# cv-core/MIT-Driverless-CV-TrainingInfra

Measured on AMD Instinct MI355X. Metric: images/sec training (YOLOv3 416^2 + RektNet 80^2), higher is better.
Workload: dtype bf16; 1 GPU; CVC-YOLOv3 yolo_baseline 416x416 classes=80, train step (fwd+bwd+Adam), 32 img/GPU; global_batch=32, parallelism=dp1, hipgraph=False, optimizer=FusedAdam

## Files before the change

### include/mdcv_hip.h

```cpp
#ifndef MDCV_HIP_H
#define MDCV_HIP_H
#ifdef __cplusplus
extern "C" {
#endif

#define MDCV_OK 0
#define MDCV_EARG (-1)
#define MDCV_F32 0
#define MDCV_BF16 1
#define MDCV_TUNED(dtype, code) (((dtype) & 0xff) | ((code) * 256))
#define MDCV_ACT_NONE 0
#define MDCV_ACT_LEAKY 1
#define MDCV_ACT_RELU 2

int mdcv_conv2d(int dtype, int mode, const void* in, int in_ldc, const void* w_packed, void* out, int out_ldc,
                const float* bias, const void* addsrc, int add_ldc, float* stats_partial,
                int B, int Hin, int Win, int Cin, int Hout, int Wout, int Nout,
                int KH, int KW, int stride, int pad, int dil, void* stream);
int mdcv_conv2d_affine_act(int dtype, const void* in, int in_ldc, const void* w_packed, void* out, int out_ldc, const float* scale,
                           const float* shift, const void* addsrc, int add_ldc, int act, float slope, int B, int Hin, int Win, int Cin,
                           int Hout, int Wout, int Nout, int KH, int KW, int stride, int pad, int dil, void* stream);
int mdcv_conv2d_dgrad_bnsums_rows(int dtype, int B, int Hin, int Win, int Cin, int Hout, int Wout, int Nout, int KH, int KW, int stride,
                                  int pad, int dil, int in_ldc);
int mdcv_conv2d_dgrad_bnsums(int dtype, const void* in, int in_ldc, const void* w_packed, void* out, int out_ldc, const void* addsrc,
// ... 162 lines not shown
int mdcv_event_destroy(void* ev);
int mdcv_probe_mfma(int blocks, int iters, float* sink, double* flops, void* stream);
int mdcv_stream_fork(void* from, void* to, int device_scope);
int mdcv_stream_fork_arm(void* from, int device_scope, void** ev_out);
int mdcv_stream_fork_wait(void* to, void* ev);
int mdcv_profile_begin(void);
int mdcv_profile_count(void);
int mdcv_profile_stop(void);
int mdcv_profile_read(int i, float* ms, char* name, int name_len);
int mdcv_graph_begin(void* stream);
int mdcv_graph_end(void* stream, void** graph_exec);
int mdcv_graph_launch(void* graph_exec, void* stream);
int mdcv_graph_destroy(void* graph_exec);

int mdcv_pw_rows(long long M, int K);
int mdcv_pw_conv_fwd(int dtype, const void* y, int ldy, const float* scale, const float* shift, const void* resid, int ldr, int act,
                     float slope, void* z_out, int ldz, const void* w_packed, const float* bias, void* out, int out_ldc,
                     float* stats_partial, long long M, int K, int N, void* stream);

int mdcv_pw_bwd_slabs(int dtype, long long M, int Cin, int Cout, int ldy, int ldx, int lddx, int ldadd, int ldfy);
int mdcv_pw_bwd(int dtype, const void* dy, int ldy, const void* x, int ldx, const void* wd_packed, void* dx, int lddx, const void* addsrc,
                int ldadd, float* ws, int slabs, const void* fy, int ldfy, const float* fscale, const float* fshift, const float* fmean, int fact,
                float fslope, float* fpartial, long long M, int Cin, int Cout, void* stream);
int mdcv_conv2d_wgrad_bnapply_ok(int dtype, int B, int Hin, int Win, int Cin, int Hout, int Wout, int Cout, int KH, int KW, int stride,
                                 int pad, int dil, int dz_ldc, int y_ldc, int x_ldc);
int mdcv_conv2d_wgrad_bnapply(int dtype, const void* dz, int dz_ldc, const void* y, int y_ldc, const float* scale, const float* shift,
                              const float* cA, const float* cB, const float* cC, int act, float slope, const void* x, int x_ldc, float* ws,
                              int splits, float* dw_oihw, int accumulate, int B, int Hin, int Win, int Cin, int Cin_real, int Hout, int Wout,
                              int Cout, int Cout_real, int KH, int KW, int stride, int pad, int dil, void* stream);
int mdcv_wgrad_reduce(const float* ws, int splits, float* dw_oihw, int accumulate, int Cout_pad, int Cout, int Cin_pad, int Cin, int KK,
                      void* stream);

int mdcv_comm_unique_id(void* id128);
int mdcv_comm_init(void** comm, int nranks, const void* id128, int rank);
int mdcv_comm_allreduce_sum(void* comm, float* buf, long long n, void* stream);
int mdcv_comm_destroy(void* comm);

#ifdef __cplusplus
}
#endif
#endif
```

### mit-driverless-cv-traininginfra_amd/csrc/pw_bwd.hip

```cpp
#include "common.h"
#include "bn_fuse.h"

struct PwbArgs {
  const void* dy; const void* x; const void* wd; void* dx; const void* addsrc; float* ws;
  int ldy, ldx, lddx, ldadd;
  int M, Cin, Cout;
  int slab_px, nslabs, slices;
  BnFuseArgs fuse;
};

namespace {

constexpr int NT = 512, NW = 8;
constexpr int BP = 32;
constexpr int NS = 64;
constexpr int T64 = 2 * 2048 + 128;
constexpr int SPITCH = 136;
typedef __attribute__((address_space(3))) void lds_void_t;
typedef __attribute__((ext_vector_type(4))) short s16x4_t;
typedef __attribute__((ext_vector_type(8))) short s16x8_t;


__device__ __forceinline__ int swz(int row) { return (row >> 1) & 2; }
__device__ __forceinline__ unsigned lds_u32(const unsigned char* p) {
  return (unsigned)(size_t)(const __attribute__((address_space(3))) unsigned char*)p;
}
__device__ __forceinline__ uint2 lds_rd64(unsigned addr) {
  uint2 v;
  asm volatile("ds_read_b64 %0, %1" : "=v"(v) : "v"(addr) : "memory");
  return v;
}
template <int OFF> __device__ __forceinline__ s16x4_t lds_tr16(unsigned addr) {
  s16x4_t v;
  asm volatile("ds_read_b64_tr_b16 %0, %1 offset:%2" : "=v"(v) : "v"(addr), "n"(OFF) : "memory");
  return v;
}

template <int CO4, int S, bool ADD, bool FUSE>
__global__ __launch_bounds__(NT) void pw_bwd_kernel(PwbArgs a) {
  constexpr int KB = 2 * CO4;
  constexpr int NX = 1 + (ADD ? 1 : 0) + (FUSE ? 1 : 0);
  constexpr int WD_BYTES = KB * 4096;
  constexpr int STG = KB * 2048 + NX * T64;
  constexpr int STAGING = WD_BYTES + S * STG;
  constexpr int DUMP = STAGING + BP * SPITCH;
  constexpr int NCHUNK = 2 * KB + 4 * NX;
  constexpr int NPW = (NCHUNK + NW - 1) / NW;
  extern __shared__ __attribute__((aligned(1024))) unsigned char smem[];

  const int xcd = (int)(blockIdx.x & 7), seq = (int)(blockIdx.x >> 3);
  const int slab = xcd + 8 * (seq / a.slices), slice = seq % a.slices;
  if (slab >= a.nslabs) return;
  const int tid = threadIdx.x, lane = tid & 63;
  const int wave = __builtin_amdgcn_readfirstlane(tid >> 6);
  const int px0 = slab * a.slab_px;
  const int px_end = min(a.M, px0 + a.slab_px);
  const int ntiles = (px_end - px0 + BP - 1) / BP;
  const int ci0 = slice * NS;

  const __amdgpu_buffer_rsrc_t rwd = __builtin_amdgcn_make_buffer_rsrc(const_cast<void*>(a.wd), 0, (unsigned)a.Cin * (unsigned)a.Cout * 2u, 0x00020000);

  const int lrow = lane >> 2, lslot = (lane & 3) ^ swz(lrow);
#define PWB_SETUP(I)                                                                                                               \
  const int c##I = wave + NW * I;                                                                                 \
  const int cc##I = c##I - 2 * KB, t##I = cc##I >> 2, b##I = (cc##I >> 1) & 1, g##I = c##I & 1;                                      \
  const bool isdy##I = c##I < 2 * KB, live##I = c##I < NCHUNK;                                                                       \
  const int k##I = isdy##I ? 0 : (t##I == 0 ? 1 : ((ADD && t##I == 1) ? 2 : 3));                      \
  const void* bp##I = k##I == 0 ? a.dy : (k##I == 1 ? a.x : (k##I == 2 ? a.addsrc : a.fuse.y));                                     \
  const unsigned ld##I = (unsigned)(k##I == 0 ? a.ldy : (k##I == 1 ? a.ldx : (k##I == 2 ? a.ldadd : a.fuse.ldy)));                  \
  const unsigned pitch##I = live##I ? ld##I * 2u : 0u;                                                                              \
  const __amdgpu_buffer_rsrc_t rs##I = __builtin_amdgcn_make_buffer_rsrc(const_cast<void*>(live##I ? bp##I : a.dy), 0,              \
                                                                         live##I ? (unsigned)px_end * ld##I * 2u : 0u, 0x00020000); \
  const int ch##I = isdy##I ? (c##I >> 1) * 32 : ci0 + b##I * 32;                                                                   \
  const unsigned voff##I = live##I ? (unsigned)(g##I * 16 + lrow) * pitch##I + (unsigned)(ch##I + lslot * 8) * 2u : 0u;             \
  const unsigned ldso##I = !live##I ? (unsigned)(DUMP - WD_BYTES)                                                                   \
                                    : (isdy##I ? (unsigned)((c##I >> 1) * 2048 + g##I * 1024)                                       \
                                               : (unsigned)(KB * 2048 + t##I * T64 + b##I * (2048 + 128) + g##I * 1024));           \
  const unsigned smul##I = live##I ? (unsigned)STG : 0u;
  PWB_SETUP(0) PWB_SETUP(1) PWB_SETUP(2) PWB_SETUP(3) PWB_SETUP(4) PWB_SETUP(5)
#undef PWB_SETUP
  static_assert(NPW <= 6, "six DMA roles per wave");
#define PWB_ISSUE_ONE(I, PROW_, SLOT_)                                                                                             \
  if constexpr (I < NPW)                                                                                                          \
    __builtin_amdgcn_raw_ptr_buffer_load_lds(rs##I, (lds_void_t*)(smem + WD_BYTES + (unsigned)(SLOT_) * smul##I + ldso##I), 16,      \
                                             (int)voff##I, (int)((PROW_) * pitch##I), 0, 0)
#define PWB_ISSUE_TILE(T_, SLOT_)                                                                                                  \
  do {                                                                                                                           \
    const unsigned prow__ = (unsigned)(px0 + (T_) * BP);                                                                         \
    PWB_ISSUE_ONE(0, prow__, SLOT_); PWB_ISSUE_ONE(1, prow__, SLOT_); PWB_ISSUE_ONE(2, prow__, SLOT_);                           \
    PWB_ISSUE_ONE(3, prow__, SLOT_); PWB_ISSUE_ONE(4, prow__, SLOT_); PWB_ISSUE_ONE(5, prow__, SLOT_);                           \
  } while (0)

#pragma unroll
  for (int i = 0; i < (4 * KB) / NW; ++i) {
    const int c = wave + NW * i, kb = c >> 2, g = c & 3;
    const unsigned vo = (unsigned)(ci0 + g * 16 + lrow) * (unsigned)a.Cout * 2u + (unsigned)(kb * 32 + lslot * 8) * 2u;
    __builtin_amdgcn_raw_ptr_buffer_load_lds(rwd, (lds_void_t*)(smem + kb * 4096 + g * 1024), 16, (int)vo, 0, 0, 0);
  }
  int issued = 0;
  for (; issued < S - 1 && issued < ntiles; ++issued) PWB_ISSUE_TILE(issued, issued);

  const int r16 = lane & 15, q4 = lane >> 4;
  const int offF = r16 * 64 + ((q4 ^ swz(r16)) << 4);
  const int cb = wave & 3, pb = wave >> 2;
  const unsigned char* const pWd = smem + (cb * 16) * 64 + offF;
  const int trow = q4 * 4 + (r16 >> 2);
  const int tsub = (r16 & 1) * 8, tq = (r16 & 3) >> 1;
  const int wc = wave >> 1, wn = wave & 1;
  const int erow = tid >> 4, ecg = tid & 15;
  const int eblk = ecg >> 3, eslot = (ecg & 7) >> 1, esub = (ecg & 1) * 8;
  const int eoff64 = eblk * (2048 + 128) + erow * 64 + ((eslot ^ swz(erow & 15)) << 4) + esub;
  bf16_t* __restrict__ dxp = reinterpret_cast<bf16_t*>(a.dx);
  const unsigned stg_wr = lds_u32(smem) + (unsigned)(STAGING + (pb * 16 + r16) * SPITCH + cb * 32 + q4 * 8);

  float fs[4], fb[4], fm[4], sg[4], sx[4];
  if constexpr (FUSE) {
#pragma unroll
    for (int e = 0; e < 4; ++e) {
      const int n = ci0 + ecg * 4 + e;
      fs[e] = a.fuse.scale[n]; fb[e] = a.fuse.shift[n]; fm[e] = a.fuse.mean[n]; sg[e] = 0.f; sx[e] = 0.f;
    }
  }

  f32x4_t accw[CO4][2];
#pragma unroll
  for (int i = 0; i < CO4; ++i)
#pragma unroll
    for (int j = 0; j < 2; ++j) accw[i][j] = f32x4_t{0.f, 0.f, 0.f, 0.f};

  int slot = 0, islot = issued % S;
  for (int t = 0; t < ntiles; ++t) {
    const int newer = issued - 1 - t;
    if (S > 2 && newer >= S - 2) asm volatile("s_waitcnt vmcnt(%0)" ::"n"((S > 2 ? S - 2 : 0) * NPW) : "memory");
    else asm volatile("s_waitcnt vmcnt(0)" ::: "memory");
    asm volatile("s_waitcnt lgkmcnt(0)" ::: "memory");
    __builtin_amdgcn_s_barrier();
    if (issued < ntiles) {
      PWB_ISSUE_TILE(issued, islot);
      ++issued;
      islot = islot + 1 == S ? 0 : islot + 1;
    }
    const unsigned char* stg = smem + WD_BYTES + slot * STG;

    {
      f32x4_t acc = f32x4_t{0.f, 0.f, 0.f, 0.f};
      const unsigned char* pB = stg + (pb * 16) * 64 + offF;
#pragma unroll
      for (int kb = 0; kb < KB; ++kb) {
        const bf16x8_t fa = *reinterpret_cast<const bf16x8_t*>(pWd + kb * 4096);
        const bf16x8_t fbv = *reinterpret_cast<const bf16x8_t*>(pB + kb * 2048);
        acc = __builtin_amdgcn_mfma_f32_16x16x32_bf16(fa, fbv, acc, 0, 0, 0);
      }
      uint2 pk;
      pk.x = pack_bf16x2(acc[0], acc[1]); pk.y = pack_bf16x2(acc[2], acc[3]);
      asm volatile("ds_write_b64 %0, %1" ::"v"(stg_wr), "v"(pk) : "memory");
    }

    {
      bf16x8_t fx[2], fd[CO4];
      const unsigned xb = lds_u32(stg) + (unsigned)(KB * 2048 + wn * (2048 + 128) + trow * 64 + tsub);
#pragma unroll
      for (int j = 0; j < 2; ++j) {
        const unsigned ad = xb + (unsigned)((((2 * j + tq) ^ swz(trow)) << 4));
        const s16x4_t lo = lds_tr16<0>(ad), hi = lds_tr16<1024>(ad);
        const s16x8_t v = {lo[0], lo[1], lo[2], lo[3], hi[0], hi[1], hi[2], hi[3]};
        fx[j] = __builtin_bit_cast(bf16x8_t, v);
      }
      const unsigned db = lds_u32(stg) + (unsigned)(trow * 64 + tsub);
#pragma unroll
      for (int i = 0; i < CO4; ++i) {
        const int gblk = wc * CO4 + i;
        const unsigned ad = db + (unsigned)((gblk >> 1) * 2048) + (unsigned)((((2 * (gblk & 1) + tq) ^ swz(trow)) << 4));
        const s16x4_t lo = lds_tr16<0>(ad), hi = lds_tr16<1024>(ad);
        const s16x8_t v = {lo[0], lo[1], lo[2], lo[3], hi[0], hi[1], hi[2], hi[3]};
        fd[i] = __builtin_bit_cast(bf16x8_t, v);
      }
      asm volatile("s_waitcnt lgkmcnt(0)" ::: "memory");
#pragma unroll
      for (int j = 0; j < 2; ++j) asm volatile("" : "+v"(fx[j]));
#pragma unroll
      for (int i = 0; i < CO4; ++i) asm volatile("" : "+v"(fd[i]));
#pragma unroll
      for (int i = 0; i < CO4; ++i)
#pragma unroll
        for (int j = 0; j < 2; ++j) accw[i][j] = __builtin_amdgcn_mfma_f32_16x16x32_bf16(fd[i], fx[j], accw[i][j], 0, 0, 0);
    }

    asm volatile("s_waitcnt lgkmcnt(0)" ::: "memory");
    __builtin_amdgcn_s_barrier();
    {
      const int p = px0 + t * BP + erow;
      const unsigned sbase = lds_u32(stg) + (unsigned)(KB * 2048 + eoff64);
      uint2 d = lds_rd64(lds_u32(smem) + (unsigned)(STAGING + erow * SPITCH + ecg * 8)), q = d, yq = d;
      if constexpr (ADD) q = lds_rd64(sbase + T64);
      if constexpr (FUSE) yq = lds_rd64(sbase + (NX - 1) * T64);
      asm volatile("s_waitcnt lgkmcnt(0)" : "+v"(d), "+v"(q), "+v"(yq)::"memory");
      float v[4];
      v[0] = __uint_as_float(d.x << 16); v[1] = __uint_as_float(d.x & 0xffff0000u);
      v[2] = __uint_as_float(d.y << 16); v[3] = __uint_as_float(d.y & 0xffff0000u);
      if constexpr (ADD) {
        v[0] += __uint_as_float(q.x << 16); v[1] += __uint_as_float(q.x & 0xffff0000u);
        v[2] += __uint_as_float(q.y << 16); v[3] += __uint_as_float(q.y & 0xffff0000u);
        d.x = pack_bf16x2(v[0], v[1]); d.y = pack_bf16x2(v[2], v[3]);
      }
      if (p < px_end) *reinterpret_cast<uint2*>(dxp + (size_t)p * a.lddx + ci0 + ecg * 4) = d;
      if constexpr (FUSE) {
        if (p < px_end) {
          float yv[4];
          yv[0] = __uint_as_float(yq.x << 16); yv[1] = __uint_as_float(yq.x & 0xffff0000u);
          yv[2] = __uint_as_float(yq.y << 16); yv[3] = __uint_as_float(yq.y & 0xffff0000u);
          v[0] = __uint_as_float(d.x << 16); v[1] = __uint_as_float(d.x & 0xffff0000u);
          v[2] = __uint_as_float(d.y << 16); v[3] = __uint_as_float(d.y & 0xffff0000u);
#pragma unroll
          for (int e = 0; e < 4; ++e) {
            const float pre = __builtin_fmaf(yv[e], fs[e], fb[e]);
// ... 26 lines not shown
      sg[e] += __shfl_xor(sg[e], 32, 64); sx[e] += __shfl_xor(sx[e], 32, 64);
    }
    asm volatile("s_waitcnt vmcnt(0) lgkmcnt(0)" ::: "memory");
    __builtin_amdgcn_s_barrier();
    float* red = reinterpret_cast<float*>(smem + WD_BYTES);
    if (lane < 16) {
#pragma unroll
      for (int e = 0; e < 4; ++e) { red[(wave * 2 + 0) * 64 + lane * 4 + e] = sg[e]; red[(wave * 2 + 1) * 64 + lane * 4 + e] = sx[e]; }
    }
    __syncthreads();
    if (tid < 128) {
      float tot = 0.f;
#pragma unroll
      for (int w = 0; w < NW; ++w) tot += red[w * 128 + tid];
      const int which = tid >> 6, c = tid & 63;
      a.fuse.partial[(size_t)(a.fuse.row_base + slab) * 2 * a.Cin + (size_t)which * a.Cin + ci0 + c] = tot;
    }
  }
}

#undef PWB_ISSUE_TILE
#undef PWB_ISSUE_ONE

template <int CO4, int S, bool ADD, bool FUSE>
int launch_pwb(const PwbArgs& a, hipStream_t st) {
  constexpr int KB = 2 * CO4, NX = 1 + (ADD ? 1 : 0) + (FUSE ? 1 : 0);
  constexpr int LDS = KB * 4096 + S * (KB * 2048 + NX * T64) + BP * SPITCH + 1024;
  static_assert(LDS <= 160 * 1024, "LDS budget");
  auto kern = pw_bwd_kernel<CO4, S, ADD, FUSE>;
  static DynLds dyn_lds;
  if (hipError_t e = mdcv_dyn_lds(dyn_lds, reinterpret_cast<const void*>(kern), LDS); e != hipSuccess) return (int)e;
  const unsigned grid = (unsigned)(8 * cdiv(a.nslabs, 8) * a.slices);
  MDCV_LAUNCH(kern, dim3(grid), dim3(NT), LDS, st, a);
  MDCV_CHECK_LAUNCH();
  return MDCV_OK;
}

template <int CO4, int S>
int launch_pwb2(const PwbArgs& a, hipStream_t st) {
  const bool add = a.addsrc != nullptr, fuse = a.fuse.y != nullptr;
  if (add) return fuse ? launch_pwb<CO4, S, true, true>(a, st) : launch_pwb<CO4, S, true, false>(a, st);
  return fuse ? launch_pwb<CO4, S, false, true>(a, st) : launch_pwb<CO4, S, false, false>(a, st);
}

int device_cus() {
  static int cus[64] = {};
  int dev = 0;
  if (hipGetDevice(&dev) != hipSuccess || dev < 0 || dev >= 64) return 256;
  if (!cus[dev]) {
    int n = 0;
    cus[dev] = (hipDeviceGetAttribute(&n, hipDeviceAttributeMultiprocessorCount, dev) == hipSuccess && n >= 8) ? n : 256;
  }
  return cus[dev];
}

int pwb_lds_bytes(int Cout) {
  const int KB = Cout / 32, S = Cout >= 512 ? 2 : 3;
  return KB * 4096 + S * (KB * 2048 + 3 * T64) + BP * SPITCH + 1024;
}

}

extern "C" {

int mdcv_pw_bwd_slabs(int dtype, long long M, int Cin, int Cout, int ldy, int ldx, int lddx, int ldadd, int ldfy) {
  if (dtype != MDCV_BF16 || M < 1) return 0;
  if (Cout != 64 && Cout != 128 && Cout != 256 && Cout != 512) return 0;
  if (Cin < 64 || (Cin & 63)) return 0;
  if ((ldy & 7) || (ldx & 7) || (lddx & 3) || (ldadd & 7) || (ldfy & 7)) return 0;
  const long long ldmax = (long long)(ldy > ldx ? ldy : ldx) > (ldadd > ldfy ? ldadd : ldfy) ? (ldy > ldx ? ldy : ldx) : (ldadd > ldfy ? ldadd : ldfy);
  if ((M + 64) * ldmax * 2 >= (1LL << 31) || (long long)Cin * Cout * 2 >= (1LL << 31)) return 0;
  const int ncu = device_cus();
  const int per_cu = (160 * 1024) / pwb_lds_bytes(Cout);
  const int slices = Cin / NS;
  const int xcd_slots = (ncu / 8) * (per_cu < 1 ? 1 : per_cu);
  int P = 8 * (xcd_slots / slices > 0 ? xcd_slots / slices : 1);
  long long spx = ((M + P - 1) / P + BP - 1) / BP * BP;
  if (spx < 4 * BP) spx = 4 * BP;
  return (int)((M + spx - 1) / spx);
}

int mdcv_pw_bwd(int dtype, const void* dy, int ldy, const void* x, int ldx, const void* wd_packed, void* dx, int lddx, const void* addsrc,
                int ldadd, float* ws, int slabs, const void* fy, int ldfy, const float* fscale, const float* fshift, const float* fmean, int fact,
                float fslope, float* fpartial, long long M, int Cin, int Cout, void* stream) {
  if (!dy || !x || !wd_packed || !dx || !ws) return MDCV_EARG;
  if (slabs < 1 || slabs != mdcv_pw_bwd_slabs(dtype, M, Cin, Cout, ldy, ldx, lddx, addsrc ? ldadd : 8, fy ? ldfy : 8)) return MDCV_EARG;
  PwbArgs a{};
  a.dy = dy; a.x = x; a.wd = wd_packed; a.dx = dx; a.addsrc = addsrc; a.ws = ws;
  a.ldy = ldy; a.ldx = ldx; a.lddx = lddx; a.ldadd = ldadd;
  a.M = (int)M; a.Cin = Cin; a.Cout = Cout;
  a.nslabs = slabs; a.slices = Cin / NS;
  a.slab_px = (int)(((M + slabs - 1) / slabs + BP - 1) / BP * BP);
  a.fuse = BnFuseArgs{};
  if (fy) {
    if (!fscale || !fshift || !fmean || !fpartial) return MDCV_EARG;
    a.fuse.y = fy; a.fuse.ldy = ldfy; a.fuse.scale = fscale; a.fuse.shift = fshift; a.fuse.mean = fmean; a.fuse.partial = fpartial;
    a.fuse.act = fact; a.fuse.slope = fact == 2 ? 0.f : fslope; a.fuse.row_base = 0;
  }
  hipStream_t st = (hipStream_t)stream;
  switch (Cout) {
    case 64: return launch_pwb2<1, 3>(a, st);
    case 128: return launch_pwb2<2, 3>(a, st);
    case 256: return launch_pwb2<4, 3>(a, st);
    case 512: return launch_pwb2<8, 2>(a, st);
  }
  return MDCV_EARG;
}

}
```

### mit-driverless-cv-traininginfra_amd/engine.py

```python
import os

import torch

from . import _lib
from ._lib import F32, BF16, ACT_NONE, ACT_LEAKY, ACT_RELU, tuned


_POISON = os.environ.get("MDCV_POISON", "0") == "1"
_REDZONE = int(os.environ.get("MDCV_REDZONE", "0"))
_RZ_BYTE = 0xA5


def _alloc(n, dtype, device, zero, plan):
    if not _REDZONE:
        t = (torch.zeros if zero else torch.empty)(n, dtype=dtype, device=device)
        if not zero and _POISON and t.is_floating_point():
            t.fill_(float("nan"))
        return t
    es = torch.empty(0, dtype=dtype).element_size()
    raw = torch.full((n * es + _REDZONE,), _RZ_BYTE, dtype=torch.uint8, device=device)
    t = raw[:n * es].view(dtype)
    if zero:
        t.zero_()
    plan.__dict__.setdefault("redzones", []).append((raw, n * es))
# ... 292 lines not shown
        self.call(self.fwd, self.L.conv2d, self.cdt, 0, x.ptr, x.ldc, cs.wf.data_ptr(), y.ptr, y.ldc,
                  cs.bias_pad.data_ptr() if cs.bias_pad is not None else None, None, 0,
                  stats_partial.data_ptr() if stats_partial is not None else None,
                  x.B, x.H, x.W, cs.cin_pad, y.H, y.W, cs.cout_pad, cs.kh, cs.kw, cs.stride, cs.pad, cs.dil)

    def emit_conv_bwd(self, cs, xnode, y_shape_act, dy, x_wgrad=None):
        L, dt = self.L, self.dtype
        x = xnode.act
        if x_wgrad is None and self._emit_pw_bwd1(cs, xnode, dy):
            return
        xw = x_wgrad if x_wgrad is not None else x
        cin_w = xw.C if x_wgrad is not None else cs.cin_pad
        if self.wgrad_after_dgrad and cs.kh == 3 and cs.stride == 1:
            self._emit_dgrad(cs, xnode, dy)
            self._emit_wgrad_single(cs, xw, dy, cin_w)
        else:
            self._emit_wgrad_single(cs, xw, dy, cin_w)
            self._emit_dgrad(cs, xnode, dy)

    wgrad_after_dgrad = False

    pw_bwd1 = True

    def _emit_pw_bwd1(self, cs, xnode, dy):
        L, dt = self.L, self.dtype
        x = xnode.act
        if not self.pw_bwd1 or dt != BF16 or not xnode.needs_grad or cs.wd is None:
            return False
        if (cs.kh, cs.kw, cs.stride, cs.pad) != (1, 1, 1, 0) or x.C != cs.cin_pad or dy.C != cs.cout_pad:
            return False
        slabs = int(L.pw_bwd_slabs(dt, x.M, cs.cin_pad, cs.cout_pad, dy.ldc, x.ldc, 8, 8, 8))
        if slabs < 1:
            return False
        out, add = self.grad_target(xnode)
        assert slabs == int(L.pw_bwd_slabs(dt, x.M, cs.cin_pad, cs.cout_pad, dy.ldc, x.ldc, out.ldc, add.ldc if add is not None else 8, 8))
        gw = self.param_grad(cs.weight)
        ws = self.f32(slabs * cs.cout_pad * cs.cin_pad, zero=False)
        args = [dt, dy.ptr, dy.ldc, x.ptr, x.ldc, cs.wd.data_ptr(), out.ptr, out.ldc, add.ptr if add is not None else None,
                add.ldc if add is not None else 0, ws.data_ptr(), slabs, None, 0, None, None, None, 0, 0.0, None, x.M, cs.cin_pad, cs.cout_pad]
        self.dgrad_entries[out.ptr] = dict(
            idx=len(self.bwd), out=out, used=False, pwb=args,
            geom=(x.B, dy.H, dy.W, cs.cout_pad, x.H, x.W, cs.cin_pad, cs.kh, cs.kw, cs.stride, cs.pad, cs.dil), head=(dy.ptr, dy.ldc))
        self.call(self.bwd, L.pw_bwd, *args)

        def wreduce(stream, ws=ws, gw=gw, slabs=slabs, cs=cs):
            return L.wgrad_reduce(ws.data_ptr(), slabs, gw.data_ptr(), 0, cs.cout_pad, cs.cout, cs.cin_pad, cs.cin, 1, stream)
        wreduce.__name__ = "conv2d_wgrad"
        wreduce.info = (x.B, x.H, x.W, cs.cin_pad, dy.H, dy.W, cs.cout_pad, 0, 1, slabs)
        self.bwd.append((wreduce, ()))
        self.pw_bwd1_count = getattr(self, "pw_bwd1_count", 0) + 1
        return True

    def _emit_wgrad_single(self, cs, xw, dy, cin_w):
        L, dt = self.L, self.dtype
        gw = self.param_grad(cs.weight)
        splits = int(L.conv2d_wgrad_splits_geom(self.wdt, xw.B, xw.H, xw.W, cin_w, dy.H, dy.W, cs.cout_pad, cs.kh, cs.kw, cs.stride, cs.pad,
                                                cs.dil, dy.ldc, xw.ldc))
        self.ws_floats = max(self.ws_floats, splits * cs.cout_pad * cs.kh * cs.kw * cin_w)
        plan = self

        def wgrad(stream, cs=cs, x=xw, dy=dy, gw=gw, splits=splits, cin_w=cin_w):
            return L.conv2d_wgrad(plan.wdt, dy.ptr, dy.ldc, x.ptr, x.ldc, plan.wgrad_ws(stream).data_ptr(), splits, gw.data_ptr(), 0,
                                  x.B, x.H, x.W, cin_w, cs.cin, dy.H, dy.W, cs.cout_pad, cs.cout, cs.kh, cs.kw,
                                  cs.stride, cs.pad, cs.dil, stream)
        wgrad.__name__ = "conv2d_wgrad"
        wgrad.info = (xw.B, xw.H, xw.W, cin_w, dy.H, dy.W, cs.cout_pad, cs.kh, cs.stride, splits)
# ... 207 lines not shown
        if not self.wgrad_bnapply or xnode.needs_grad or self.dtype != BF16 or cs.bias is not None:
            return False
        geom = (x.B, x.H, x.W, cs.cin_pad, y.H, y.W, cs.cout_pad, cs.kh, cs.kw, cs.stride, cs.pad, cs.dil)
        if not int(L.conv2d_wgrad_bnapply_ok(self.wdt, *geom, dout.ldc, y.ldc, x.ldc)):
            return False
        self.emit_bn_act_bwd(dout, y, bs, act, slope, apply=False)
        gw = self.param_grad(cs.weight)
        sdt = _lib.tuned(self.dtype, 20000 + 768) if self.tune_wgrad == 0 else self.wdt
        splits = int(L.conv2d_wgrad_splits_geom(sdt, *geom, dout.ldc, x.ldc))
        self.ws_floats = max(self.ws_floats, splits * cs.cout_pad * cs.kh * cs.kw * cs.cin_pad)
        plan = self
        n = lambda t: t.data_ptr()

        def wgrad(stream):
            return L.conv2d_wgrad_bnapply(plan.wdt, dout.ptr, dout.ldc, y.ptr, y.ldc, n(bs.scale), n(bs.shift), n(bs.cA), n(bs.cB), n(bs.cC), act,
                                          float(slope), x.ptr, x.ldc, plan.wgrad_ws(stream).data_ptr(), splits, gw.data_ptr(), 0, x.B, x.H, x.W,
                                          cs.cin_pad, cs.cin, y.H, y.W, cs.cout_pad, cs.cout, cs.kh, cs.kw, cs.stride, cs.pad, cs.dil, stream)
        wgrad.__name__ = "conv2d_wgrad"
        wgrad.info = (x.B, x.H, x.W, cs.cin_pad, y.H, y.W, cs.cout_pad, cs.kh, cs.stride, splits)
        self.bwd.append((wgrad, ()))
        self.first_conv_fused = True
        return True

    fuse_bn = True

    fuse_skip = 141
    fuse_max_rows = 4096
    fuse_max_rows_s2 = 1 << 16

    def _fuse_pays(self, geom):
        B, dyH, dyW, cdy, xH, xW, cdx, kh, kw, stride, pad, dil = geom
        px = B * xH * xW
        k = self.fuse_skip
        if kh == 3 and stride == 1:
            if 50000 <= px < 100000:
                return not (k & 1)
            if 20000 <= px < 50000:
                return not (k & 2)
            if px >= 300000:
                return not (k & 32)
            if px < 20000:
                return not (k & 256)
        if kh == 1:
            if px >= 300000:
                return not (k & 4)
            if 50000 <= px < 100000:
# ... 4 lines not shown
                return not (k & 512)
        if stride == 2 and 300000 <= px < 1000000:
            return not (k & 8)
        if stride == 2 and px < 300000:
            return not (k & 128)
        return True

    def _fuse_bn_sums(self, dout, y, bs, act, slope, dgamma, dbeta):
        if not self.fuse_bn or self.dtype != BF16:
            return False
        e = self.dgrad_entries.get(dout.ptr)
        if e is None or e["used"]:
            return False
        o = e["out"]
        if (o.M, o.C, o.ldc) != (dout.M, dout.C, dout.ldc) or (y.M, y.C) != (dout.M, dout.C):
            return False
        for fn, args in self.bwd[e["idx"] + 1:]:
            if dout.ptr in args:
                return False
        L, dt = self.L, self.dtype
        pwb = e.get("pwb")
        g = e["geom"]
        if pwb is not None:
            rows = int(pwb[11])
            partial = self.f32(rows * 2 * y.C, zero=False)
            a2 = list(pwb)
            a2[12:20] = [y.ptr, y.ldc, bs.scale.data_ptr(), bs.shift.data_ptr(), bs.mean.data_ptr(), act, float(slope), partial.data_ptr()]
            assert self.bwd[e["idx"]][0] is L.pw_bwd
            self.bwd[e["idx"]] = (L.pw_bwd, tuple(a2))
        else:
            s2_shift = bool(L.conv2d_dgrad_s2_form_ok(self.cdt, *g, e["head"][1]))
            if not s2_shift and not self._fuse_pays(g):
                return False
            rows = int(L.conv2d_dgrad_bnsums_rows(self.cdt, *g, e["head"][1]))
            if rows <= 0 or rows > (self.fuse_max_rows_s2 if s2_shift else self.fuse_max_rows):
                return False
            assert self.bwd[e["idx"]][0] is L.conv2d
            partial = self.f32(rows * 2 * y.C, zero=False)
            h = e["head"]
            self.bwd[e["idx"]] = (L.conv2d_dgrad_bnsums, (self.cdt, h[0], h[1], h[2], h[3], h[4], h[5], h[6], *e["geom"], y.ptr, y.ldc,
                                                          bs.scale.data_ptr(), bs.shift.data_ptr(), bs.mean.data_ptr(), act, float(slope),
                                                          partial.data_ptr()))
        e["used"] = True
        self.call(self.bwd, L.bn_bwd_finalize_rows, partial.data_ptr(), rows, y.C, float(y.M), bs.bn.weight.data_ptr(),
                  bs.mean.data_ptr(), bs.invstd.data_ptr(), dgamma.data_ptr(), dbeta.data_ptr(), bs.cA.data_ptr(), bs.cB.data_ptr(),
                  bs.cC.data_ptr())
        self.fused_bn += 1
        return True

    def finish_pack(self, position=0):
        import struct
        rec = b"".join(struct.pack("<QQQiiiiiiiiQQ", cs.weight.data_ptr(), cs.wf.data_ptr(), cs.wd.data_ptr() if cs.wd is not None else 0,
# ... 131 lines not shown
```

### mit-driverless-cv-traininginfra_amd/netplan.py

```python
import ctypes
import os

import torch

from . import _lib
from .engine import Plan, side_stream


_EVAL_FUSE = True


class _NetPlan(Plan):

    @classmethod
    def begin(cls, owner, device, bn_train, B, C, H, W, use_graph):
        plan = cls(device, owner.precision, bn_train, grad_sink=owner._grad_view)
        plan.owner = owner
        plan.grad_offset = lambda p: owner._goff[id(p)][0]
        plan.use_graph = use_graph
        plan.pre = []
        xin, plan.in_holder = plan.emit_input(B, C, H, W)
        plan.pre.append(plan.fwd.pop())
        plan.targets = None
        return plan, xin
# ... 87 lines not shown
                rc = fn(*args, ss)
                used = True
            else:
                if role == 1:
                    L.check(L.stream_fork_arm(st, self.fork_device_scope, ctypes.byref(ev)), "stream_fork_arm")
                    armed = True
                rc = fn(*args, st)
            if rc:
                if armed:
                    L.stream_fork_wait(ss, ev)
                raise _lib.MdcvError(f"{getattr(fn, '__name__', fn)} returned {rc}")
        if pending:
            L.check(fork(st, ss, self.fork_device_scope), "stream_fork")
            flush()
            used = True
        if used:
            L.check(fork(ss, st, self.fork_device_scope), "stream_fork")

    fork_on_dispatch = True
    defer_slab_reduce = True

    def _classify_bwd(self):
        L = self.L
        single = (L.bn_act_bwd_apply, L.pw_bwd)
        n = len(self.bwd)
        roles = [2 if getattr(fn, "__name__", "") == "conv2d_wgrad" else 0 for fn, _ in self.bwd]
        if self.defer_slab_reduce:
            for i, (fn, _) in enumerate(self.bwd):
                info = getattr(fn, "info", None)
                if roles[i] == 2 and info is not None and len(info) > 7 and info[7] == 0:
                    roles[i] = 3
        if self.fork_on_dispatch:
            for i in range(n - 1):
                if roles[i] == 0 and roles[i + 1] == 2 and any(self.bwd[i][0] is f for f in single):
                    roles[i] = 1
        return roles

    def run_backward(self, gout):
        self.gscale.copy_(gout.reshape(-1)[:self.gscale.numel()], non_blocking=True)
        if self.use_graph:
            self._graphed("bwd")
        else:
            self.run_bwd_list()


class FlatParamsMixin:

# ... 162 lines not shown
```

### mit-driverless-cv-traininginfra_amd/yolo/lower.py

```python
from collections import namedtuple
from dataclasses import dataclass

import torch

from .. import _lib, netplan
from ..engine import Act, TNode, ConvSpec, BnSpec, pad8, ACT_NONE, ACT_LEAKY, ACT_RELU


def _res(i, v):
    return i + v if v < 0 else v


def _route_sources(i, d):
    return [_res(i, int(t)) for t in d["layers"].split(",")]


Layout = namedtuple("Layout", "users shp concat dest")


def analyse(defs, mods, cin, H, W):
    users = [[] for _ in defs]
    for i, d in enumerate(defs):
        k = d["type"]
        if k in ("convolutional", "upsample", "maxpool", "yolo") and i > 0:
# ... 160 lines not shown
    if fuse:
        cx.fused_into[i + 1] = z
    else:
        cx.outs[i] = z
    return ConvBn(cs, bs, x, y, z, rnode, act_code, slope)


@dataclass
class ConvBn:
    cs: ConvSpec
    bs: BnSpec
    x: TNode
    y: Act
    z: TNode
    resid: TNode
    act_code: int
    slope: float

    def backward(self, plan):
        if self.z.gstate == "none":
            return
        if self.resid is not None:
            plan.grad_identity(self.resid, self.z.grad)
        if not plan.emit_first_conv_bwd(self.z.grad, self.y, self.bs, self.act_code, self.slope, self.cs, self.x):
            dy = plan.emit_bn_act_bwd(self.z.grad, self.y, self.bs, self.act_code, self.slope)
            plan.emit_conv_bwd(self.cs, self.x, self.y, dy)


def lower_shortcut(cx, i, d):
    if i in cx.fused_into:
        cx.done(i, cx.fused_into[i])
        return None
    a, b = cx.outs[i - 1], cx.outs[_res(i, int(d["from"]))]
    z = TNode(cx.out_act(i), name="short%d" % i)
    cx.plan.emit_add(cx.plan.fwd, a.act, b.act, z.act)
    cx.done(i, z)
    return Shortcut(a, b, z)


@dataclass
class Shortcut:
    a: TNode
    b: TNode
    z: TNode

    def backward(self, plan):
        if self.z.gstate == "none":
# ... 149 lines not shown
```

Measured before the change: 2493 images/sec.

## Fuse BN-activation backward apply into pointwise conv dgrad kernel

```diff
diff --git a/include/mdcv_hip.h b/include/mdcv_hip.h
--- a/include/mdcv_hip.h
+++ b/include/mdcv_hip.h
@@ -208,6 +208,11 @@
 int mdcv_pw_bwd(int dtype, const void* dy, int ldy, const void* x, int ldx, const void* wd_packed, void* dx, int lddx, const void* addsrc,
                 int ldadd, float* ws, int slabs, const void* fy, int ldfy, const float* fscale, const float* fshift, const float* fmean, int fact,
                 float fslope, float* fpartial, long long M, int Cin, int Cout, void* stream);
+int mdcv_pw_bwd_bnapply_slabs(int dtype, long long M, int Cin, int Cout, int lddz, int ldy, int ldx, int lddx, int ldadd, int ldfy);
+int mdcv_pw_bwd_bnapply(int dtype, const void* dz, int lddz, const void* y, int ldy, const float* scale, const float* shift, const float* cA,
+                        const float* cB, const float* cC, int act, float slope, const void* x, int ldx, const void* wd_packed, void* dx, int lddx,
+                        const void* addsrc, int ldadd, float* ws, int slabs, const void* fy, int ldfy, const float* fscale, const float* fshift,
+                        const float* fmean, int fact, float fslope, float* fpartial, long long M, int Cin, int Cout, void* stream);
 int mdcv_conv2d_wgrad_bnapply_ok(int dtype, int B, int Hin, int Win, int Cin, int Hout, int Wout, int Cout, int KH, int KW, int stride,
                                  int pad, int dil, int dz_ldc, int y_ldc, int x_ldc);
 int mdcv_conv2d_wgrad_bnapply(int dtype, const void* dz, int dz_ldc, const void* y, int y_ldc, const float* scale, const float* shift,
diff --git a/mit-driverless-cv-traininginfra_amd/csrc/pw_bwd.hip b/mit-driverless-cv-traininginfra_amd/csrc/pw_bwd.hip
--- a/mit-driverless-cv-traininginfra_amd/csrc/pw_bwd.hip
+++ b/mit-driverless-cv-traininginfra_amd/csrc/pw_bwd.hip
@@ -7,6 +7,9 @@
   int M, Cin, Cout;
   int slab_px, nslabs, slices;
   BnFuseArgs fuse;
+  const void* by; int ldby;
+  const float* bscale; const float* bshift; const float* bcA; const float* bcB; const float* bcC;
+  int bact; float bslope;
 };
 
 namespace {
@@ -36,15 +39,20 @@
   return v;
 }
 
-template <int CO4, int S, bool ADD, bool FUSE>
+template <int CO4, int S, bool ADD, bool FUSE, bool BNA>
 __global__ __launch_bounds__(NT) void pw_bwd_kernel(PwbArgs a) {
   constexpr int KB = 2 * CO4;
   constexpr int NX = 1 + (ADD ? 1 : 0) + (FUSE ? 1 : 0);
   constexpr int WD_BYTES = KB * 4096;
-  constexpr int STG = KB * 2048 + NX * T64;
+  constexpr int XOFF = (BNA ? 2 : 1) * KB * 2048;
+  constexpr int STG = XOFF + NX * T64;
   constexpr int STAGING = WD_BYTES + S * STG;
   constexpr int DUMP = STAGING + BP * SPITCH;
-  constexpr int NCHUNK = 2 * KB + 4 * NX;
+  constexpr int P2 = 2 * KB;
+  constexpr int NCHUNK = (BNA ? 2 : 1) * P2 + 4 * NX;
+  constexpr bool SMALL = BNA && P2 < 8;
+  constexpr int NTR = SMALL ? 1 : P2 / NW;
+  static_assert(!BNA || SMALL || P2 % NW == 0, "a wave owns whole (dz, by) piece pairs");
   constexpr int NPW = (NCHUNK + NW - 1) / NW;
   extern __shared__ __attribute__((aligned(1024))) unsigned char smem[];
 
@@ -63,19 +71,24 @@
   const int lrow = lane >> 2, lslot = (lane & 3) ^ swz(lrow);
 #define PWB_SETUP(I)                                                                                                               \
   const int c##I = wave + NW * I;                                                                                 \
-  const int cc##I = c##I - 2 * KB, t##I = cc##I >> 2, b##I = (cc##I >> 1) & 1, g##I = c##I & 1;                                      \
-  const bool isdy##I = c##I < 2 * KB, live##I = c##I < NCHUNK;                                                                       \
-  const int k##I = isdy##I ? 0 : (t##I == 0 ? 1 : ((ADD && t##I == 1) ? 2 : 3));                      \
-  const void* bp##I = k##I == 0 ? a.dy : (k##I == 1 ? a.x : (k##I == 2 ? a.addsrc : a.fuse.y));                                     \
-  const unsigned ld##I = (unsigned)(k##I == 0 ? a.ldy : (k##I == 1 ? a.ldx : (k##I == 2 ? a.ldadd : a.fuse.ldy)));                  \
+  const bool isdz##I = SMALL ? c##I < 4 : c##I < P2;                                                     \
+  const bool isby##I = BNA && (SMALL ? (c##I >= 8 && c##I < 12) : (c##I >= P2 && c##I < 2 * P2));                                    \
+  const bool isdy##I = isdz##I || isby##I;                                                                                          \
+  const int di##I = isby##I ? c##I - (SMALL ? 8 : P2) : c##I;                              \
+  const int cc##I = c##I - (!BNA ? P2 : (SMALL ? (c##I < 8 ? 4 : 8) : 2 * P2));                                                       \
+  const int t##I = cc##I >> 2, b##I = (cc##I >> 1) & 1, g##I = c##I & 1;                                                             \
+  const bool live##I = c##I < NCHUNK;                                                                                               \
+  const int k##I = isdz##I ? 0 : (isby##I ? 4 : (t##I == 0 ? 1 : ((ADD && t##I == 1) ? 2 : 3)));    \
+  const void* bp##I = k##I == 0 ? a.dy : (k##I == 1 ? a.x : (k##I == 2 ? a.addsrc : (k##I == 3 ? a.fuse.y : a.by)));                 \
+  const unsigned ld##I = (unsigned)(k##I == 0 ? a.ldy : (k##I == 1 ? a.ldx : (k##I == 2 ? a.ldadd : (k##I == 3 ? a.fuse.ldy : a.ldby)))); \
   const unsigned pitch##I = live##I ? ld##I * 2u : 0u;                                                                              \
   const __amdgpu_buffer_rsrc_t rs##I = __builtin_amdgcn_make_buffer_rsrc(const_cast<void*>(live##I ? bp##I : a.dy), 0,              \
                                                                          live##I ? (unsigned)px_end * ld##I * 2u : 0u, 0x00020000); \
-  const int ch##I = isdy##I ? (c##I >> 1) * 32 : ci0 + b##I * 32;                                                                   \
+  const int ch##I = isdy##I ? (di##I >> 1) * 32 : ci0 + b##I * 32;                                                                  \
   const unsigned voff##I = live##I ? (unsigned)(g##I * 16 + lrow) * pitch##I + (unsigned)(ch##I + lslot * 8) * 2u : 0u;             \
   const unsigned ldso##I = !live##I ? (unsigned)(DUMP - WD_BYTES)                                                                   \
-                                    : (isdy##I ? (unsigned)((c##I >> 1) * 2048 + g##I * 1024)                                       \
-                                               : (unsigned)(KB * 2048 + t##I * T64 + b##I * (2048 + 128) + g##I * 1024));           \
+                                    : (isdy##I ? (unsigned)((isby##I ? KB * 2048 : 0) + (di##I >> 1) * 2048 + g##I * 1024)           \
+                                               : (unsigned)(XOFF + t##I * T64 + b##I * (2048 + 128) + g##I * 1024));                \
   const unsigned smul##I = live##I ? (unsigned)STG : 0u;
   PWB_SETUP(0) PWB_SETUP(1) PWB_SETUP(2) PWB_SETUP(3) PWB_SETUP(4) PWB_SETUP(5)
 #undef PWB_SETUP
@@ -113,6 +126,29 @@
   bf16_t* __restrict__ dxp = reinterpret_cast<bf16_t*>(a.dx);
   const unsigned stg_wr = lds_u32(smem) + (unsigned)(STAGING + (pb * 16 + r16) * SPITCH + cb * 32 + q4 * 8);
 
+  const bool tr_wave = !SMALL || wave < 4;
+  const int tr_row = (wave & 1) * 16 + lrow;
+  float ts[BNA ? NTR : 1][8], tb[BNA ? NTR : 1][8], tA[BNA ? NTR : 1][8], tB[BNA ? NTR : 1][8], tC[BNA ? NTR : 1][8];
+  if constexpr (BNA) {
+    if (tr_wave) {
+#pragma unroll
+      for (int j = 0; j < NTR; ++j) {
+        const int c0 = ((wave + NW * j) >> 1) * 32 + lslot * 8;
+#pragma unroll
+        for (int q = 0; q < 2; ++q) {
+          const float4 v0 = *reinterpret_cast<const float4*>(a.bscale + c0 + 4 * q), v1 = *reinterpret_cast<const float4*>(a.bshift + c0 + 4 * q);
+          const float4 v2 = *reinterpret_cast<const float4*>(a.bcA + c0 + 4 * q), v3 = *reinterpret_cast<const float4*>(a.bcB + c0 + 4 * q);
+          const float4 v4 = *reinterpret_cast<const float4*>(a.bcC + c0 + 4 * q);
+          ts[j][4 * q] = v0.x; ts[j][4 * q + 1] = v0.y; ts[j][4 * q + 2] = v0.z; ts[j][4 * q + 3] = v0.w;
+          tb[j][4 * q] = v1.x; tb[j][4 * q + 1] = v1.y; tb[j][4 * q + 2] = v1.z; tb[j][4 * q + 3] = v1.w;
+          tA[j][4 * q] = v2.x; tA[j][4 * q + 1] = v2.y; tA[j][4 * q + 2] = v2.z; tA[j][4 * q + 3] = v2.w;
+          tB[j][4 * q] = v3.x; tB[j][4 * q + 1] = v3.y; tB[j][4 * q + 2] = v3.z; tB[j][4 * q + 3] = v3.w;
+          tC[j][4 * q] = v4.x; tC[j][4 * q + 1] = v4.y; tC[j][4 * q + 2] = v4.z; tC[j][4 * q + 3] = v4.w;
+        }
+      }
+    }
+  }
+
   float fs[4], fb[4], fm[4], sg[4], sx[4];
   if constexpr (FUSE) {
 #pragma unroll
@@ -133,6 +169,34 @@
     const int newer = issued - 1 - t;
     if (S > 2 && newer >= S - 2) asm volatile("s_waitcnt vmcnt(%0)" ::"n"((S > 2 ? S - 2 : 0) * NPW) : "memory");
     else asm volatile("s_waitcnt vmcnt(0)" ::: "memory");
+    if constexpr (BNA) {
+      if (tr_wave) {
+        typedef unsigned u32x4_t __attribute__((ext_vector_type(4)));
+        const bool row_live = px0 + t * BP + tr_row < px_end;
+        u32x4_t rd[NTR], ry[NTR];
+        unsigned ad[NTR];
+#pragma unroll
+        for (int j = 0; j < NTR; ++j) {
+          ad[j] = lds_u32(smem) + (unsigned)(WD_BYTES + slot * STG + ((wave + NW * j) >> 1) * 2048 + (wave & 1) * 1024 + lane * 16);
+          asm volatile("ds_read_b128 %0, %1" : "=v"(rd[j]) : "v"(ad[j]) : "memory");
+          asm volatile("ds_read_b128 %0, %1 offset:%2" : "=v"(ry[j]) : "v"(ad[j]), "n"(KB * 2048) : "memory");
+        }
+        asm volatile("s_waitcnt lgkmcnt(0)" ::: "memory");
+#pragma unroll
+        for (int j = 0; j < NTR; ++j) {
+          asm volatile("" : "+v"(rd[j]), "+v"(ry[j]));
+          float d[8], v[8], o[8];
+          ET<bf16_t>::unpack(make_uint4(rd[j][0], rd[j][1], rd[j][2], rd[j][3]), d);
+          ET<bf16_t>::unpack(make_uint4(ry[j][0], ry[j][1], ry[j][2], ry[j][3]), v);
+#pragma unroll
+          for (int e = 0; e < 8; ++e)
+            o[e] = row_live ? mdcv_bn_bwd_dy(d[e], v[e], ts[j][e], tb[j][e], tA[j][e], tB[j][e], tC[j][e], a.bact, a.bslope) : 0.f;
+          const uint4 qo = ET<bf16_t>::pack(o);
+          const u32x4_t wo = {qo.x, qo.y, qo.z, qo.w};
+          asm volatile("ds_write_b128 %0, %1" ::"v"(ad[j]), "v"(wo) : "memory");
+        }
+      }
+    }
     asm volatile("s_waitcnt lgkmcnt(0)" ::: "memory");
     __builtin_amdgcn_s_barrier();
     if (issued < ntiles) {
@@ -158,7 +222,7 @@
 
     {
       bf16x8_t fx[2], fd[CO4];
-      const unsigned xb = lds_u32(stg) + (unsigned)(KB * 2048 + wn * (2048 + 128) + trow * 64 + tsub);
+      const unsigned xb = lds_u32(stg) + (unsigned)(XOFF + wn * (2048 + 128) + trow * 64 + tsub);
 #pragma unroll
       for (int j = 0; j < 2; ++j) {
         const unsigned ad = xb + (unsigned)((((2 * j + tq) ^ swz(trow)) << 4));
@@ -190,7 +254,7 @@
     __builtin_amdgcn_s_barrier();
     {
       const int p = px0 + t * BP + erow;
-      const unsigned sbase = lds_u32(stg) + (unsigned)(KB * 2048 + eoff64);
+      const unsigned sbase = lds_u32(stg) + (unsigned)(XOFF + eoff64);
       uint2 d = lds_rd64(lds_u32(smem) + (unsigned)(STAGING + erow * SPITCH + ecg * 8)), q = d, yq = d;
       if constexpr (ADD) q = lds_rd64(sbase + T64);
       if constexpr (FUSE) yq = lds_rd64(sbase + (NX - 1) * T64);
@@ -263,12 +327,16 @@
 #undef PWB_ISSUE_TILE
 #undef PWB_ISSUE_ONE
 
-template <int CO4, int S, bool ADD, bool FUSE>
+constexpr int pwb_lds(int KB, int S, int nx, bool bna) { return KB * 4096 + S * ((bna ? 2 : 1) * KB * 2048 + nx * T64) + BP * SPITCH + 1024; }
+constexpr int PWB_LDS_MAX = 160 * 1024;
+constexpr int pwb_stages(int KB, int nx, bool bna) { return pwb_lds(KB, 3, nx, bna) <= PWB_LDS_MAX && KB < 16 ? 3 : 2; }
+
+template <int CO4, bool ADD, bool FUSE, bool BNA>
 int launch_pwb(const PwbArgs& a, hipStream_t st) {
-  constexpr int KB = 2 * CO4, NX = 1 + (ADD ? 1 : 0) + (FUSE ? 1 : 0);
-  constexpr int LDS = KB * 4096 + S * (KB * 2048 + NX * T64) + BP * SPITCH + 1024;
-  static_assert(LDS <= 160 * 1024, "LDS budget");
-  auto kern = pw_bwd_kernel<CO4, S, ADD, FUSE>;
+  constexpr int KB = 2 * CO4, NX = 1 + (ADD ? 1 : 0) + (FUSE ? 1 : 0), S = pwb_stages(KB, NX, BNA);
+  constexpr int LDS = pwb_lds(KB, S, NX, BNA);
+  static_assert(LDS <= PWB_LDS_MAX, "LDS budget");
+  auto kern = pw_bwd_kernel<CO4, S, ADD, FUSE, BNA>;
   static DynLds dyn_lds;
   if (hipError_t e = mdcv_dyn_lds(dyn_lds, reinterpret_cast<const void*>(kern), LDS); e != hipSuccess) return (int)e;
   const unsigned grid = (unsigned)(8 * cdiv(a.nslabs, 8) * a.slices);
@@ -277,11 +345,11 @@
   return MDCV_OK;
 }
 
-template <int CO4, int S>
+template <int CO4, bool BNA>
 int launch_pwb2(const PwbArgs& a, hipStream_t st) {
   const bool add = a.addsrc != nullptr, fuse = a.fuse.y != nullptr;
-  if (add) return fuse ? launch_pwb<CO4, S, true, true>(a, st) : launch_pwb<CO4, S, true, false>(a, st);
-  return fuse ? launch_pwb<CO4, S, false, true>(a, st) : launch_pwb<CO4, S, false, false>(a, st);
+  if (add) return fuse ? launch_pwb<CO4, true, true, BNA>(a, st) : launch_pwb<CO4, true, false, BNA>(a, st);
+  return fuse ? launch_pwb<CO4, false, true, BNA>(a, st) : launch_pwb<CO4, false, false, BNA>(a, st);
 }
 
 int device_cus() {
@@ -298,6 +366,28 @@
 int pwb_lds_bytes(int Cout) {
   const int KB = Cout / 32, S = Cout >= 512 ? 2 : 3;
   return KB * 4096 + S * (KB * 2048 + 3 * T64) + BP * SPITCH + 1024;
+}
+int pwb_bna_lds_bytes(int Cout) {
+  const int KB = Cout / 32;
+  const int lds = pwb_lds(KB, pwb_stages(KB, 3, true), 3, true);
+  return lds <= PWB_LDS_MAX ? lds : 0;
+}
+
+int fill_pwb(PwbArgs& a, const void* dy, int ldy, const void* x, int ldx, const void* wd_packed, void* dx, int lddx, const void* addsrc, int ldadd,
+             float* ws, int slabs, const void* fy, int ldfy, const float* fscale, const float* fshift, const float* fmean, int fact, float fslope,
+             float* fpartial, long long M, int Cin, int Cout) {
+  a.dy = dy; a.x = x; a.wd = wd_packed; a.dx = dx; a.addsrc = addsrc; a.ws = ws;
+  a.ldy = ldy; a.ldx = ldx; a.lddx = lddx; a.ldadd = ldadd;
+  a.M = (int)M; a.Cin = Cin; a.Cout = Cout;
+  a.nslabs = slabs; a.slices = Cin / NS;
+  a.slab_px = (int)(((M + slabs - 1) / slabs + BP - 1) / BP * BP);
+  a.fuse = BnFuseArgs{};
+  if (fy) {
+    if (!fscale || !fshift || !fmean || !fpartial) return MDCV_EARG;
+    a.fuse.y = fy; a.fuse.ldy = ldfy; a.fuse.scale = fscale; a.fuse.shift = fshift; a.fuse.mean = fmean; a.fuse.partial = fpartial;
+    a.fuse.act = fact; a.fuse.slope = fact == 2 ? 0.f : fslope; a.fuse.row_base = 0;
+  }
+  return MDCV_OK;
 }
 
 }
@@ -327,25 +417,45 @@
   if (!dy || !x || !wd_packed || !dx || !ws) return MDCV_EARG;
   if (slabs < 1 || slabs != mdcv_pw_bwd_slabs(dtype, M, Cin, Cout, ldy, ldx, lddx, addsrc ? ldadd : 8, fy ? ldfy : 8)) return MDCV_EARG;
   PwbArgs a{};
-  a.dy = dy; a.x = x; a.wd = wd_packed; a.dx = dx; a.addsrc = addsrc; a.ws = ws;
-  a.ldy = ldy; a.ldx = ldx; a.lddx = lddx; a.ldadd = ldadd;
-  a.M = (int)M; a.Cin = Cin; a.Cout = Cout;
-  a.nslabs = slabs; a.slices = Cin / NS;
-  a.slab_px = (int)(((M + slabs - 1) / slabs + BP - 1) / BP * BP);
-  a.fuse = BnFuseArgs{};
-  if (fy) {
-    if (!fscale || !fshift || !fmean || !fpartial) return MDCV_EARG;
-    a.fuse.y = fy; a.fuse.ldy = ldfy; a.fuse.scale = fscale; a.fuse.shift = fshift; a.fuse.mean = fmean; a.fuse.partial = fpartial;
-    a.fuse.act = fact; a.fuse.slope = fact == 2 ? 0.f : fslope; a.fuse.row_base = 0;
-  }
+  if (const int rc = fill_pwb(a, dy, ldy, x, ldx, wd_packed, dx, lddx, addsrc, ldadd, ws, slabs, fy, ldfy, fscale, fshift, fmean, fact, fslope, fpartial,
+                              M, Cin, Cout); rc != MDCV_OK) return rc;
   hipStream_t st = (hipStream_t)stream;
   switch (Cout) {
-    case 64: return launch_pwb2<1, 3>(a, st);
-    case 128: return launch_pwb2<2, 3>(a, st);
-    case 256: return launch_pwb2<4, 3>(a, st);
-    case 512: return launch_pwb2<8, 2>(a, st);
+    case 64: return launch_pwb2<1, false>(a, st);
+    case 128: return launch_pwb2<2, false>(a, st);
+    case 256: return launch_pwb2<4, false>(a, st);
+    case 512: return launch_pwb2<8, false>(a, st);
   }
   return MDCV_EARG;
 }
 
-}
+int mdcv_pw_bwd_bnapply_slabs(int dtype, long long M, int Cin, int Cout, int lddz, int ldy, int ldx, int lddx, int ldadd, int ldfy) {
+  const int slabs = mdcv_pw_bwd_slabs(dtype, M, Cin, Cout, lddz, ldx, lddx, ldadd, ldfy);
+  if (slabs < 1) return 0;
+  if ((ldy & 7) || (M + 64) * (long long)ldy * 2 >= (1LL << 31)) return 0;
+  const int lds = pwb_bna_lds_bytes(Cout);
+  if (!lds || PWB_LDS_MAX / lds < PWB_LDS_MAX / pwb_lds_bytes(Cout)) return 0;
+  return slabs;
+}
+
+int mdcv_pw_bwd_bnapply(int dtype, const void* dz, int lddz, const void* y, int ldy, const float* scale, const float* shift, const float* cA,
+                        const float* cB, const float* cC, int act, float slope, const void* x, int ldx, const void* wd_packed, void* dx, int lddx,
+                        const void* addsrc, int ldadd, float* ws, int slabs, const void* fy, int ldfy, const float* fscale, const float* fshift,
+                        const float* fmean, int fact, float fslope, float* fpartial, long long M, int Cin, int Cout, void* stream) {
+  if (!dz || !y || !scale || !shift || !cA || !cB || !cC || !x || !wd_packed || !dx || !ws) return MDCV_EARG;
+  if (slabs < 1 || slabs != mdcv_pw_bwd_bnapply_slabs(dtype, M, Cin, Cout, lddz, ldy, ldx, lddx, addsrc ? ldadd : 8, fy ? ldfy : 8)) return MDCV_EARG;
+  PwbArgs a{};
+  if (const int rc = fill_pwb(a, dz, lddz, x, ldx, wd_packed, dx, lddx, addsrc, ldadd, ws, slabs, fy, ldfy, fscale, fshift, fmean, fact, fslope, fpartial,
+                              M, Cin, Cout); rc != MDCV_OK) return rc;
+  a.by = y; a.ldby = ldy; a.bscale = scale; a.bshift = shift; a.bcA = cA; a.bcB = cB; a.bcC = cC;
+  a.bact = act; a.bslope = act == 2 ? 0.f : slope;
+  hipStream_t st = (hipStream_t)stream;
+  switch (Cout) {
+    case 64: return launch_pwb2<1, true>(a, st);
+    case 128: return launch_pwb2<2, true>(a, st);
+    case 256: return launch_pwb2<4, true>(a, st);
+  }
+  return MDCV_EARG;
+}
+
+}
diff --git a/mit-driverless-cv-traininginfra_amd/engine.py b/mit-driverless-cv-traininginfra_amd/engine.py
--- a/mit-driverless-cv-traininginfra_amd/engine.py
+++ b/mit-driverless-cv-traininginfra_amd/engine.py
@@ -338,26 +338,41 @@
 
     pw_bwd1 = True
 
-    def _emit_pw_bwd1(self, cs, xnode, dy):
+    def _pw_bwd1_slabs(self, cs, xnode, dy, bna_y=None, lddx=8, ldadd=8):
         L, dt = self.L, self.dtype
         x = xnode.act
         if not self.pw_bwd1 or dt != BF16 or not xnode.needs_grad or cs.wd is None:
-            return False
+            return 0
         if (cs.kh, cs.kw, cs.stride, cs.pad) != (1, 1, 1, 0) or x.C != cs.cin_pad or dy.C != cs.cout_pad:
-            return False
-        slabs = int(L.pw_bwd_slabs(dt, x.M, cs.cin_pad, cs.cout_pad, dy.ldc, x.ldc, 8, 8, 8))
+            return 0
+        if bna_y is not None:
+            return int(L.pw_bwd_bnapply_slabs(dt, x.M, cs.cin_pad, cs.cout_pad, dy.ldc, bna_y.ldc, x.ldc, lddx, ldadd, 8))
+        return int(L.pw_bwd_slabs(dt, x.M, cs.cin_pad, cs.cout_pad, dy.ldc, x.ldc, lddx, ldadd, 8))
+
+    def _emit_pw_bwd1(self, cs, xnode, dy, bna=None):
+        L, dt = self.L, self.dtype
+        x = xnode.act
+        by = bna[0] if bna is not None else None
+        slabs = self._pw_bwd1_slabs(cs, xnode, dy, by)
         if slabs < 1:
             return False
         out, add = self.grad_target(xnode)
-        assert slabs == int(L.pw_bwd_slabs(dt, x.M, cs.cin_pad, cs.cout_pad, dy.ldc, x.ldc, out.ldc, add.ldc if add is not None else 8, 8))
+        assert slabs == self._pw_bwd1_slabs(cs, xnode, dy, by, out.ldc, add.ldc if add is not None else 8)
         gw = self.param_grad(cs.weight)
         ws = self.f32(slabs * cs.cout_pad * cs.cin_pad, zero=False)
-        args = [dt, dy.ptr, dy.ldc, x.ptr, x.ldc, cs.wd.data_ptr(), out.ptr, out.ldc, add.ptr if add is not None else None,
-                add.ldc if add is not None else 0, ws.data_ptr(), slabs, None, 0, None, None, None, 0, 0.0, None, x.M, cs.cin_pad, cs.cout_pad]
+        head = [dt, dy.ptr, dy.ldc]
+        fn = L.pw_bwd
+        if bna is not None:
+            y, bs, act, slope = bna
+            n = lambda t: t.data_ptr()
+            head += [y.ptr, y.ldc, n(bs.scale), n(bs.shift), n(bs.cA), n(bs.cB), n(bs.cC), act, float(slope)]
+            fn = L.pw_bwd_bnapply
+        args = head + [x.ptr, x.ldc, cs.wd.data_ptr(), out.ptr, out.ldc, add.ptr if add is not None else None,
+                       add.ldc if add is not None else 0, ws.data_ptr(), slabs, None, 0, None, None, None, 0, 0.0, None, x.M, cs.cin_pad, cs.cout_pad]
         self.dgrad_entries[out.ptr] = dict(
-            idx=len(self.bwd), out=out, used=False, pwb=args,
+            idx=len(self.bwd), out=out, used=False, pwb=args, pwb_fn=fn, pwb_at=len(head) + 8,
             geom=(x.B, dy.H, dy.W, cs.cout_pad, x.H, x.W, cs.cin_pad, cs.kh, cs.kw, cs.stride, cs.pad, cs.dil), head=(dy.ptr, dy.ldc))
-        self.call(self.bwd, L.pw_bwd, *args)
+        self.call(self.bwd, fn, *args)
 
         def wreduce(stream, ws=ws, gw=gw, slabs=slabs, cs=cs):
             return L.wgrad_reduce(ws.data_ptr(), slabs, gw.data_ptr(), 0, cs.cout_pad, cs.cout, cs.cin_pad, cs.cin, 1, stream)
@@ -611,6 +626,19 @@
         self.first_conv_fused = True
         return True
 
+    pw_bwd_bnapply = True
+
+    def emit_pw_bwd_bnapply(self, dout, y, bs, act, slope, cs, xnode):
+        if not self.pw_bwd_bnapply or cs.bias is not None or cs.cout != cs.cout_pad or (y.M, y.C) != (dout.M, dout.C):
+            return False
+        if self._pw_bwd1_slabs(cs, xnode, dout, y) < 1:
+            return False
+        self.emit_bn_act_bwd(dout, y, bs, act, slope, apply=False)
+        ok = self._emit_pw_bwd1(cs, xnode, dout, bna=(y, bs, act, slope))
+        assert ok
+        self.pw_bwd_bnapply_count = getattr(self, "pw_bwd_bnapply_count", 0) + 1
+        return True
+
     fuse_bn = True
 
     fuse_skip = 141
@@ -661,12 +689,13 @@
         pwb = e.get("pwb")
         g = e["geom"]
         if pwb is not None:
-            rows = int(pwb[11])
+            at = e["pwb_at"]
+            rows = int(pwb[at])
             partial = self.f32(rows * 2 * y.C, zero=False)
             a2 = list(pwb)
-            a2[12:20] = [y.ptr, y.ldc, bs.scale.data_ptr(), bs.shift.data_ptr(), bs.mean.data_ptr(), act, float(slope), partial.data_ptr()]
-            assert self.bwd[e["idx"]][0] is L.pw_bwd
-            self.bwd[e["idx"]] = (L.pw_bwd, tuple(a2))
+            a2[at + 1:at + 9] = [y.ptr, y.ldc, bs.scale.data_ptr(), bs.shift.data_ptr(), bs.mean.data_ptr(), act, float(slope), partial.data_ptr()]
+            assert self.bwd[e["idx"]][0] is e["pwb_fn"]
+            self.bwd[e["idx"]] = (e["pwb_fn"], tuple(a2))
         else:
             s2_shift = bool(L.conv2d_dgrad_s2_form_ok(self.cdt, *g, e["head"][1]))
             if not s2_shift and not self._fuse_pays(g):
diff --git a/mit-driverless-cv-traininginfra_amd/netplan.py b/mit-driverless-cv-traininginfra_amd/netplan.py
--- a/mit-driverless-cv-traininginfra_amd/netplan.py
+++ b/mit-driverless-cv-traininginfra_amd/netplan.py
@@ -133,7 +133,7 @@
 
     def _classify_bwd(self):
         L = self.L
-        single = (L.bn_act_bwd_apply, L.pw_bwd)
+        single = (L.bn_act_bwd_apply, L.pw_bwd, L.pw_bwd_bnapply)
         n = len(self.bwd)
         roles = [2 if getattr(fn, "__name__", "") == "conv2d_wgrad" else 0 for fn, _ in self.bwd]
         if self.defer_slab_reduce:
diff --git a/mit-driverless-cv-traininginfra_amd/yolo/lower.py b/mit-driverless-cv-traininginfra_amd/yolo/lower.py
--- a/mit-driverless-cv-traininginfra_amd/yolo/lower.py
+++ b/mit-driverless-cv-traininginfra_amd/yolo/lower.py
@@ -206,7 +206,8 @@
             return
         if self.resid is not None:
             plan.grad_identity(self.resid, self.z.grad)
-        if not plan.emit_first_conv_bwd(self.z.grad, self.y, self.bs, self.act_code, self.slope, self.cs, self.x):
+        args = (self.z.grad, self.y, self.bs, self.act_code, self.slope, self.cs, self.x)
+        if not plan.emit_first_conv_bwd(*args) and not plan.emit_pw_bwd_bnapply(*args):
             dy = plan.emit_bn_act_bwd(self.z.grad, self.y, self.bs, self.act_code, self.slope)
             plan.emit_conv_bwd(self.cs, self.x, self.y, dy)
 
```

After: 2406 images/sec. 3.5% lower.
